# MaurizioFD/RecSys2019_DeepLearning_Evaluation

Hardware: AMD Instinct MI355X
Metric: BPR-MF SGD samples/sec (k=128, batch 1000) + ItemKNN cosine build sec on ML-20M-shaped URM (higher is better)
Workload: dtype f32; 1 GPU; BPR-MF epoch (139 mini-batches x 1000 on-device samples), k=128, sgd, on synthetic ml20m URM 138493x26744 nnz=20001422; replicas (one independent model per GPU); batch_size=1000, n_factors=128, parallelism=replicas x1

## Files before the change

recsys2019_deeplearning_evaluation_amd/csrc/mf_batch.cuh:

```cuda
#pragma once

namespace mi355rec {
namespace {

template <class T, int VEC> struct alignas(sizeof(T) * VEC) Chunk { T v[VEC]; };

template <class T, int VEC>
__device__ __forceinline__ Chunk<T, VEC> load_chunk(const T *row, int chunk, bool ok) {
    Chunk<T, VEC> r = *reinterpret_cast<const Chunk<T, VEC> *>(row + (size_t)(ok ? chunk : 0) * VEC);
#pragma unroll
    for (int e = 0; e < VEC; ++e) r.v[e] = ok ? r.v[e] : (T)0;
    return r;
}

template <class T, class P> __device__ __forceinline__ void adam_powers(const P &p, long long t, T &pw1, T &pw2) {
    pw1 = (T)1;
    pw2 = (T)1;
    if (p.sgd_mode == MI355REC_ADAM) {
        pw1 = (T)(1.0 - pow(p.beta_1_d, (double)t));
        pw2 = (T)(1.0 - pow(p.beta_2_d, (double)t));
    }
}

template <class T> struct MuRequest { MuState<T> st; T part; };

template <class T>
__device__ __forceinline__ MuRequest<T> global_bias_request(const MfParams<T> &p, const int prev, int lane) {
    MuRequest<T> r;
    r.st = p.mu_state[prev];
    r.part = p.mu_acc[prev * MU_SLOTS + lane];
    return r;
}

template <class T>
__device__ __forceinline__ T global_bias_finish(const MfParams<T> &p, MuRequest<T> r, long long gb, const int at, bool writer, int lane) {
    const int cur = at % 3, nxt = (at + 1) % 3;
    MuState<T> st = r.st;
    const T sum = wave_sum(r.part);
    if (gb > 0) {
        T pw1, pw2;
        adam_powers(p, gb, pw1, pw2);
        const T step = adapt_cell(p, sum * p.inv_batch, st.c1, st.c2, pw1, pw2);
        st.mu += p.lr * step;
    }
    if (writer) {
        if (lane == 0) p.mu_state[cur] = st;
        p.mu_acc[nxt * MU_SLOTS + lane] = (T)0;
    }
    return st.mu;
}

template <class T>
__device__ __forceinline__ T global_bias_at(const MfParams<T> &p, long long gb, const int at, bool writer, int lane) {
    return global_bias_finish(p, global_bias_request(p, (at + 2) % 3, lane), gb, at, writer, lane);
}

template <class T, int VEC, int KI, bool BPR> struct Rows {
    Chunk<T, VEC> A[KI], B[KI], C[BPR ? KI : 1];
    T bu, bi;
};

template <class T, int VEC, int LPR, int KI, bool BPR>
__device__ __forceinline__ Rows<T, VEC, KI, BPR> load_rows(const MfParams<T> &p, const int4 rec, int li, const bool (&cok)[KI],
                                                           bool bias) {
    Rows<T, VEC, KI, BPR> r;
    const int k = p.k;
    const T *Wu = ((rec.w >> 2) & 1 ? p.U1 : p.U0) + (size_t)rec.x * k;
    const T *Hi = ((rec.w >> 3) & 1 ? p.V1 : p.V0) + (size_t)rec.y * k;
    const T *Hj = ((rec.w >> 4) & 1 ? p.V1 : p.V0) + (size_t)(BPR ? rec.z : 0) * k;
#pragma unroll
    for (int c = 0; c < KI; ++c) {
        r.A[c] = load_chunk<T, VEC>(Wu, c * LPR + li, cok[c]);
        r.B[c] = load_chunk<T, VEC>(Hi, c * LPR + li, cok[c]);
        if (BPR) r.C[c] = load_chunk<T, VEC>(Hj, c * LPR + li, cok[c]);
    }
    r.bu = (T)0;
    r.bi = (T)0;
    if (bias) {
        r.bu = ((rec.w >> 2) & 1 ? p.bu1 : p.bu0)[rec.x];
        r.bi = ((rec.w >> 3) & 1 ? p.bi1 : p.bi0)[rec.y];
    }
    return r;
}

template <int ALGO, class T, int VEC, int LPR, int KI, bool ARGS_HERE>
__device__ __forceinline__ void mf_batch_body(const MfParams<T> &p, const int batch_local, const int wg, const int wv, const int tpb,
                                              const TaskHeader *hdr, const int4 *slot, const bool stamps) {
    constexpr int G = 64 / LPR;
    constexpr bool BPR = ALGO == MI355REC_MF_BPR;
    using Ch = Chunk<T, VEC>;
    using R = Rows<T, VEC, KI, BPR>;
    const int lane = threadIdx.x & 63;
    const unsigned long long tk0 = stamps ? stamp() : 0ull;
    const TaskHeader *hp = hdr + min(wv, tpb - 1);
    const int8v hd = *reinterpret_cast<const int8v *>(hp);
    int4 slot_rec = make_int4(0, 0, 0, 0);
    if constexpr (BPR && G > 1) slot_rec = slot[(size_t)min(wv, tpb - 1) * 3 + max(lane / LPR - 1, 0)];
    if constexpr (ARGS_HERE) {
        asm volatile("" ::"s"(p.ticks), "s"(p.use_bias), "s"(p.sgd_mode), "s"(p.state), "s"(p.mu_state), "s"(p.mu_acc), "s"(p.k), "s"(p.U0),
                     "s"(p.U1), "s"(p.V0), "s"(p.V1), "s"(p.recs));
    }
    const bool bias = !BPR && p.use_bias;
    long long gb = batch_local;
    long long batch_base = 0;
    MuRequest<T> mu_req;
    mu_req.st = MuState<T>{};
    mu_req.part = (T)0;
    if constexpr (!BPR) {
        int zero;
        asm volatile("v_mov_b32 %0, 0" : "=v"(zero));
        batch_base = (&p.state->batch_base)[zero];
        mu_req = global_bias_request(p, (batch_local + 2) % 3 + zero, lane);
    }
    if constexpr (!ARGS_HERE) asm volatile("" ::"s"(p.k), "s"(p.U0), "s"(p.U1), "s"(p.V0), "s"(p.V1), "s"(p.recs));
    if constexpr (BPR) {
        if (p.sgd_mode == MI355REC_ADAM) gb += p.state->batch_base;
    } else {
        gb += batch_base;
    }
    const int4 h0 = make_int4(hd[0], hd[1], hd[2], hd[3]), h1 = make_int4(hd[4], hd[5], hd[6], hd[7]);
    const bool active = (h0.y & LEN_MASK) != 0 && wv < tpb;
    __shared__ T s_mu[4];
    __shared__ T s_wide[4][LPR * KI * VEC];
    __shared__ T s_wide_bias[4];
    T mu_term = (T)0;
    T mu_eff = (T)0;
    unsigned long long tk1 = 0, tk2 = 0, tk3 = 0, tk4 = 0, tk5 = 0;
    if (p.ticks) tk1 = stamp();
    if (bias && !active) mu_eff = global_bias_finish(p, mu_req, gb, batch_local, wv == 0, lane);
    if (active) {
        const int entry = h0.x, len = h0.y & LEN_MASK, own_par = (unsigned)h0.y >> 31, start = h0.z;
        const bool wide = (h0.y & META_WIDE) != 0;
        const int part = (h0.y >> 28) & 3;
        const int base = wide ? part * G : 0, step = wide ? 4 * G : G;
        const int g = lane / LPR, li = lane % LPR;
        const int k = p.k, chunks = k / VEC;
        bool cok[KI];
#pragma unroll
        for (int c = 0; c < KI; ++c) cok[c] = c * LPR + li < chunks;
        const int iters = len > base ? (len - base + step - 1) / step : 0;
        int4 rec = h1;
        const bool pair = BPR && G > 1 && h0.w == 1;
        T sg_first = (T)0;
        if (BPR && G > 1 && h0.w == 1) {
            if (g != 0) rec = slot_rec;
        } else if (G > 1 && len > 1) {
            const int4 r = p.recs[start + min(base + g, len - 1)];
            if (g != 0) rec = r;
        }
        const int4 rec_first = rec;
        int4 rec_n = rec;
        if (iters > 1) rec_n = p.recs[start + min(base + step + g, len - 1)];
        R rows = load_rows<T, VEC, LPR, KI, BPR>(p, rec, li, cok, bias);
        if (bias) mu_eff = global_bias_finish(p, mu_req, gb, batch_local, wv == 0, lane);
        T pw1, pw2;
        adam_powers(p, gb + 1, pw1, pw2);

        Ch acc[KI], own[KI];
#pragma unroll
        for (int c = 0; c < KI; ++c)
#pragma unroll
            for (int e = 0; e < VEC; ++e) { acc[c].v[e] = (T)0; own[c].v[e] = (T)0; }
        T bias_acc = (T)0, own_bias = (T)0;
        double loss = 0.0;

        for (int it = 0; it < iters; ++it) {
            const int idx = base + it * step + g;
            const bool valid = idx < len;
            int4 rec_nn = rec_n;
            if (it + 2 < iters) rec_nn = p.recs[start + min(idx + 2 * step, len - 1)];
            R rows_n = rows;
            if (it + 1 < iters) rows_n = load_rows<T, VEC, LPR, KI, BPR>(p, rec_n, li, cok, bias);

            const int role = rec.w & 3;
            T dot = (T)0;
#pragma unroll
            for (int c = 0; c < KI; ++c)
#pragma unroll
                for (int e = 0; e < VEC; ++e)
                    dot = fused_add(rows.A[c].v[e], BPR ? diff_of(rows.B[c].v[e], rows.C[c].v[e]) : rows.B[c].v[e], dot);
            dot = group_sum<LPR>(dot);
            if (p.ticks && it == 0) {
                asm volatile("" ::"v"(dot));
                tk2 = stamp();
            }
            if (BPR) {
                const T x = dot;
                const T sg = sigmoid_of_minus(x);
                if (it == 0) sg_first = sg;
                if (valid && role == ROLE_U && li == 0) loss += (double)x * (double)x;
#pragma unroll
                for (int c = 0; c < KI; ++c)
#pragma unroll
                    for (int e = 0; e < VEC; ++e) {
                        const T a = rows.A[c].v[e], b = rows.B[c].v[e], cc = rows.C[c].v[e];
                        const T gU = grad_term(sg, diff_of(b, cc), p.user_reg, a);
                        const T gI = grad_term(sg, a, p.positive_reg, b);
                        const T gJ = grad_term(sg, -a, p.negative_reg, cc);
                        const T gr = role == ROLE_U ? gU : (role == ROLE_I ? gI : gJ);
                        acc[c].v[e] += valid ? gr : (T)0;
                        if (it == 0) own[c].v[e] = role == ROLE_U ? a : (role == ROLE_I ? b : cc);
                    }
            } else {
                T pred = dot;
                if (bias) pred += mu_eff + rows.bu + rows.bi;
                const T err = (T)__int_as_float(rec.z) - pred;
                if (valid && role == ROLE_U) {
                    if (li == 0) loss += (double)err * (double)err;
                    if (bias) mu_term += err - p.bias_reg * mu_eff;
                }
                if (bias && valid) bias_acc += err - p.bias_reg * (role == ROLE_U ? rows.bu : rows.bi);
                if (it == 0) own_bias = role == ROLE_U ? rows.bu : rows.bi;
#pragma unroll
                for (int c = 0; c < KI; ++c)
#pragma unroll
                    for (int e = 0; e < VEC; ++e) {
                        const T a = rows.A[c].v[e], b = rows.B[c].v[e];
                        const T gU = grad_term(err, b, p.user_reg, a);
                        const T gI = grad_term(err, a, p.positive_reg, b);
                        const T gr = role == ROLE_U ? gU : gI;
                        acc[c].v[e] += valid ? gr : (T)0;
                        if (it == 0) own[c].v[e] = role == ROLE_U ? a : b;
                    }
            }
            rec = rec_n;
            rec_n = rec_nn;
            rows = rows_n;
        }
        if (G > 1 && !pair) {
#pragma unroll
            for (int c = 0; c < KI; ++c)
#pragma unroll
                for (int e = 0; e < VEC; ++e) acc[c].v[e] = cross_group_sum<LPR>(acc[c].v[e]);
            if (bias) bias_acc = cross_group_sum<LPR>(bias_acc);
        }
        if (bias) {
            mu_term = li == 0 ? mu_term : (T)0;
            mu_term = wave_sum(mu_term);
        }
        if (li == 0 && loss != 0.0) atomicAdd(&p.loss_slots[wv * 4 + g], loss);
        if (p.ticks) tk3 = stamp();
        if (wide) {
            if (g == 0) {
#pragma unroll
                for (int c = 0; c < KI; ++c)
#pragma unroll
                    for (int e = 0; e < VEC; ++e) s_wide[part][(c * VEC + e) * LPR + li] = acc[c].v[e];
                if (li == 0) s_wide_bias[part] = bias_acc;
            }
            __syncthreads();
            if (part == 0 && g == 0) {
#pragma unroll
                for (int c = 0; c < KI; ++c)
#pragma unroll
                    for (int e = 0; e < VEC; ++e) {
                        const int at = (c * VEC + e) * LPR + li;
                        acc[c].v[e] = ((s_wide[0][at] + s_wide[1][at]) + s_wide[2][at]) + s_wide[3][at];
                    }
                bias_acc = ((s_wide_bias[0] + s_wide_bias[1]) + s_wide_bias[2]) + s_wide_bias[3];
            }
        }
        if ((g == 0 || pair) && (!wide || part == 0)) {
            const int own_entry = pair ? rec_first.x : entry;
            const int own_buf = pair ? (rec_first.w >> 2) & 1 : own_par;
            const bool is_item = own_entry >= p.n_users;
            const int row = is_item ? own_entry - p.n_users : own_entry;
            T *Wn = (is_item ? (own_buf ? p.V0 : p.V1) : (own_buf ? p.U0 : p.U1)) + (size_t)row * k;
            T *c1 = (is_item ? p.c1V : p.c1U) + (size_t)row * k, *c2 = (is_item ? p.c2V : p.c2U) + (size_t)row * k;
#pragma unroll
            for (int c = 0; c < KI; ++c) {
                if (!cok[c]) continue;
                const size_t at = (size_t)(c * LPR + li) * VEC;
                Ch m1, m2, out;
                if (p.sgd_mode != MI355REC_SGD) m1 = *reinterpret_cast<const Ch *>(c1 + at);
                if (p.sgd_mode == MI355REC_ADAM) m2 = *reinterpret_cast<const Ch *>(c2 + at);
#pragma unroll
                for (int e = 0; e < VEC; ++e) {
                    const T gm = mean_of(acc[c].v[e], p.inv_batch);
                    const T step = adapt_cell(p, gm, m1.v[e], m2.v[e], pw1, pw2);
                    out.v[e] = moved(own[c].v[e], p.lr, step);
                }
                *reinterpret_cast<Ch *>(Wn + at) = out;
                if (p.sgd_mode != MI355REC_SGD) *reinterpret_cast<Ch *>(c1 + at) = m1;
                if (p.sgd_mode == MI355REC_ADAM) *reinterpret_cast<Ch *>(c2 + at) = m2;
            }
            if (bias && li == 0) {
                T *bn = is_item ? (own_buf ? p.bi0 : p.bi1) : (own_buf ? p.bu0 : p.bu1);
                T *b1 = is_item ? p.c1_bi : p.c1_bu, *b2 = is_item ? p.c2_bi : p.c2_bu;
                const T step = adapt(p, bias_acc * p.inv_batch, b1, b2, (size_t)row, pw1, pw2);
                bn[row] = own_bias + p.lr * step;
            }
        }
        if (p.ticks) tk4 = stamp();
        const int also = BPR && (len == 1 || pair) ? (rec_first.w >> 5) & 3 : 0;
        if (BPR && also) {
#pragma unroll
            for (int e = 1; e <= 2; ++e) {
                if (!(also & e) || !(pair || g == e % G)) continue;
                const int item = e == 1 ? rec_first.y : rec_first.z;
                const int cur = (rec_first.w >> (e == 1 ? 3 : 4)) & 1;
                T *Wn = (cur ? p.V0 : p.V1) + (size_t)item * k;
                T *c1 = p.c1V + (size_t)item * k, *c2 = p.c2V + (size_t)item * k;
#pragma unroll
                for (int c = 0; c < KI; ++c) {
                    if (!cok[c]) continue;
                    const size_t at = (size_t)(c * LPR + li) * VEC;
                    Ch m1, m2, out;
                    if (p.sgd_mode != MI355REC_SGD) m1 = *reinterpret_cast<const Ch *>(c1 + at);
                    if (p.sgd_mode == MI355REC_ADAM) m2 = *reinterpret_cast<const Ch *>(c2 + at);
#pragma unroll
                    for (int v = 0; v < VEC; ++v) {
                        const T a = rows.A[c].v[v], b = rows.B[c].v[v], cc = rows.C[c].v[v];
                        const T gr = e == 1 ? grad_term(sg_first, a, p.positive_reg, b) : grad_term(sg_first, -a, p.negative_reg, cc);
                        const T gm = mean_of((T)0 + gr, p.inv_batch);
                        const T step = adapt_cell(p, gm, m1.v[v], m2.v[v], pw1, pw2);
                        out.v[v] = moved(e == 1 ? b : cc, p.lr, step);
                    }
                    *reinterpret_cast<Ch *>(Wn + at) = out;
                    if (p.sgd_mode != MI355REC_SGD) *reinterpret_cast<Ch *>(c1 + at) = m1;
                    if (p.sgd_mode == MI355REC_ADAM) *reinterpret_cast<Ch *>(c2 + at) = m2;
                }
            }
        }
    }
    if (p.ticks) tk5 = stamp();
    if (bias) {
        if (lane == 0) s_mu[threadIdx.x >> 6] = mu_term;
        __syncthreads();
        if (threadIdx.x == 0) {
            const T sum = (s_mu[0] + s_mu[1]) + (s_mu[2] + s_mu[3]);
            if (sum != (T)0) atomicAdd(&p.mu_acc[(batch_local % 3) * MU_SLOTS + (wg & (MU_SLOTS - 1))], sum);
        }
    }
    if (p.ticks && lane == 0 && wv < tpb) {
        unsigned long long *o = p.ticks + (size_t)wv * 8;
        o[0] = tk0; o[1] = tk1; o[2] = tk2; o[3] = tk3; o[4] = stamp(); o[5] = (unsigned long long)(h0.y & LEN_MASK);
        o[6] = tk4; o[7] = tk5;
    }
}

template <int ALGO, class T, int VEC, int LPR, int KI, bool PLAIN_SGD>
__global__ __launch_bounds__(256) void mf_batch_kernel(const TaskHeader *hdr, const int4 *slot, const int tasks_per_batch, const int wg_base,
                                                       const int wg_stride, const int stamps, const MfParams<T> p, const int batch_local) {
    if constexpr (PLAIN_SGD) __builtin_assume(p.sgd_mode == MI355REC_SGD);
    const int wv = __builtin_amdgcn_readfirstlane((blockIdx.x * wg_stride + wg_base) * 4 + (threadIdx.x >> 6));
    mf_batch_body<ALGO, T, VEC, LPR, KI, true>(p, batch_local, blockIdx.x, wv, tasks_per_batch, hdr, slot, stamps != 0);
}

template <class P> __device__ __forceinline__ P *as_global(P *q) {
    const unsigned long long bits = (unsigned long long)q;
    return (P *)(__attribute__((address_space(1))) P *)bits;
}
template <class T> __device__ __forceinline__ void globalize(MfParams<T> &p) {
    p.indptr = as_global(p.indptr); p.indices = as_global(p.indices); p.data = as_global(p.data);
    p.U0 = as_global(p.U0); p.U1 = as_global(p.U1); p.V0 = as_global(p.V0); p.V1 = as_global(p.V1);
    p.bu0 = as_global(p.bu0); p.bu1 = as_global(p.bu1); p.bi0 = as_global(p.bi0); p.bi1 = as_global(p.bi1);
    p.c1U = as_global(p.c1U); p.c2U = as_global(p.c2U); p.c1V = as_global(p.c1V); p.c2V = as_global(p.c2V);
    p.c1_bu = as_global(p.c1_bu); p.c2_bu = as_global(p.c2_bu); p.c1_bi = as_global(p.c1_bi); p.c2_bi = as_global(p.c2_bi);
    p.mu_state = as_global(p.mu_state); p.mu_acc = as_global(p.mu_acc);
    p.loss_slots = as_global(p.loss_slots); p.state = as_global(p.state);
    p.su = as_global(p.su); p.si = as_global(p.si); p.sj = as_global(p.sj); p.sr = as_global(p.sr);
    p.tasks = as_global(p.tasks); p.recs = as_global(p.recs); p.ticks = as_global(p.ticks); p.used = as_global(p.used);
    p.slot_recs = as_global(p.slot_recs);
}

template <int ALGO, class T, int VEC, int LPR, int KI, bool PLAIN_SGD>
__global__ __launch_bounds__(256, (PLAIN_SGD && ALGO == MI355REC_MF_BPR && sizeof(T) == 4 && LPR == 32) ? 6 : 1) void mf_group_batch_kernel(const MfParams<T> *__restrict__ table, const int batch_local) {
    MfParams<T> p = table[blockIdx.y];
    globalize(p);
    if constexpr (PLAIN_SGD) __builtin_assume(p.sgd_mode == MI355REC_SGD);
    const int used = p.used ? p.used[batch_local] : p.tasks_per_batch;
    const TaskHeader *hdr = p.tasks + (size_t)batch_local * p.tasks_per_batch;
    const int4 *slot = p.slot_recs + (size_t)batch_local * p.slot_rec_stride;
    for (int wg = blockIdx.x; wg * 4 < used; wg += gridDim.x) {
        const int wv = __builtin_amdgcn_readfirstlane((wg * p.wg_stride + p.wg_base) * 4 + (threadIdx.x >> 6));
        mf_batch_body<ALGO, T, VEC, LPR, KI, false>(p, batch_local, wg, wv, p.tasks_per_batch, hdr, slot, p.ticks != nullptr);
    }
}
__device__ __forceinline__ void globalize(FastSchedParams &f) {
    f.su = as_global(f.su); f.si = as_global(f.si); f.sj = as_global(f.sj); f.sr = as_global(f.sr);
    f.touched = as_global(f.touched); f.par = as_global(f.par); f.sorted_slot = as_global(f.sorted_slot); f.qtask = as_global(f.qtask);
    f.used = as_global(f.used); f.tasks = as_global(f.tasks); f.recs = as_global(f.recs); f.slot_recs = as_global(f.slot_recs);
}
template <int ALGO, class T>
__global__ __launch_bounds__(256) void mf_group_sample_kernel(const MfParams<T> *__restrict__ table) {
    MfParams<T> p = table[blockIdx.y];
    globalize(p);
    mf_sample_body<ALGO, T>(p);
}
template <class T>
__global__ void mf_group_epoch_advance_kernel(const MfParams<T> *table, const int n_models) {
    const int m = blockIdx.x * blockDim.x + threadIdx.x;
    if (m < n_models) table[m].state->epoch += 1;
}
__global__ __launch_bounds__(SCHED_THREADS) void mf_group_sched_sort_kernel(const FastSchedParams *__restrict__ table) {
    FastSchedParams f = table[blockIdx.y];
    globalize(f);
    mf_sched_sort_body(f, blockIdx.x);
}
__global__ __launch_bounds__(256) void mf_group_sched_emit_kernel(const FastSchedParams *__restrict__ table) {
    FastSchedParams f = table[blockIdx.z];
    globalize(f);
    mf_sched_emit_body(f);
}
__global__ __launch_bounds__(256) void mf_group_sched_finish_kernel(const FastSchedParams *__restrict__ table) {
    FastSchedParams f = table[blockIdx.y];
    globalize(f);
    mf_sched_finish_body(f);
}

template <int ALGO, class T>
__global__ __launch_bounds__(256) void mf_batch_generic_kernel(const MfParams<T> p, const int batch_local) {
    constexpr bool BPR = ALGO == MI355REC_MF_BPR;
    constexpr int KMAX_REG = 8;
    const int lane = threadIdx.x & 63;
    const int wv = __builtin_amdgcn_readfirstlane((blockIdx.x * p.wg_stride + p.wg_base) * 4 + (threadIdx.x >> 6));
    const TaskHeader *hp = p.tasks + ((size_t)batch_local * p.tasks_per_batch + min(wv, p.tasks_per_batch - 1));
    const int4 h0 = *reinterpret_cast<const int4 *>(hp);
    const bool active = (h0.y & LEN_MASK) != 0 && wv < p.tasks_per_batch;
    const bool bias = !BPR && p.use_bias;
    __shared__ T s_mu[4];
    T mu_term = (T)0;
    if (active || bias) {
        const long long gb = p.state->batch_base + batch_local;
        T mu_eff = (T)0;
        if (bias) mu_eff = global_bias_at(p, gb, batch_local, wv == 0, lane);
        if (active) {
            const int entry = h0.x, len = h0.y & LEN_MASK, own_par = (unsigned)h0.y >> 31, start = h0.z;
            const int k = p.k;
            T pw1, pw2;
            adam_powers(p, gb + 1, pw1, pw2);
            T acc[KMAX_REG];
#pragma unroll
            for (int c = 0; c < KMAX_REG; ++c) acc[c] = (T)0;
            T bias_acc = (T)0;
            double loss = 0.0;
            for (int idx = 0; idx < len; ++idx) {
                const int4 rec = idx == 0 ? hp->rec0 : p.recs[start + idx];
                const int role = rec.w & 3;
                const T *Wu = ((rec.w >> 2) & 1 ? p.U1 : p.U0) + (size_t)rec.x * k;
                const T *Hi = ((rec.w >> 3) & 1 ? p.V1 : p.V0) + (size_t)rec.y * k;
                const T *Hj = ((rec.w >> 4) & 1 ? p.V1 : p.V0) + (size_t)(BPR ? rec.z : 0) * k;
                T dot = (T)0;
                for (int f = lane; f < k; f += 64) dot += BPR ? Wu[f] * (Hi[f] - Hj[f]) : Wu[f] * Hi[f];
                dot = wave_sum(dot);
                if (BPR) {
                    const T sg = sigmoid_of_minus(dot);
                    if (role == ROLE_U) loss += (double)dot * (double)dot;
#pragma unroll
                    for (int c = 0; c < KMAX_REG; ++c) {
                        const int f = lane + 64 * c;
                        if (f < k) {
                            const T a = Wu[f], b = Hi[f], cc = Hj[f];
                            acc[c] += role == ROLE_U ? sg * (b - cc) - p.user_reg * a
                                                     : (role == ROLE_I ? sg * a - p.positive_reg * b : sg * (-a) - p.negative_reg * cc);
                        }
                    }
                } else {
                    T bu_v = (T)0, bi_v = (T)0;
                    if (bias) {
                        bu_v = ((rec.w >> 2) & 1 ? p.bu1 : p.bu0)[rec.x];
                        bi_v = ((rec.w >> 3) & 1 ? p.bi1 : p.bi0)[rec.y];
                    }
                    const T err = __int_as_float(rec.z) - (dot + (bias ? mu_eff + bu_v + bi_v : (T)0));
                    if (role == ROLE_U) {
                        loss += (double)err * (double)err;
                        if (bias) mu_term += err - p.bias_reg * mu_eff;
                    }
                    if (bias) bias_acc += err - p.bias_reg * (role == ROLE_U ? bu_v : bi_v);
#pragma unroll
                    for (int c = 0; c < KMAX_REG; ++c) {
                        const int f = lane + 64 * c;
                        if (f < k) {
                            const T a = Wu[f], b = Hi[f];
                            acc[c] += role == ROLE_U ? err * b - p.user_reg * a : err * a - p.positive_reg * b;
                        }
                    }
                }
            }
            if (lane == 0 && loss != 0.0) p.loss_slots[wv * 4] += loss;
            const bool is_item = entry >= p.n_users;
            const int row = is_item ? entry - p.n_users : entry;
            const T *Wo = (is_item ? (own_par ? p.V1 : p.V0) : (own_par ? p.U1 : p.U0)) + (size_t)row * k;
            T *Wn = (is_item ? (own_par ? p.V0 : p.V1) : (own_par ? p.U0 : p.U1)) + (size_t)row * k;
            T *c1 = is_item ? p.c1V : p.c1U, *c2 = is_item ? p.c2V : p.c2U;
#pragma unroll
            for (int c = 0; c < KMAX_REG; ++c) {
                const int f = lane + 64 * c;
                if (f < k) {
                    const T step = adapt(p, acc[c] * p.inv_batch, c1, c2, (size_t)row * k + f, pw1, pw2);
                    Wn[f] = Wo[f] + p.lr * step;
                }
            }
            if (bias && lane == 0) {
                const T *bo = is_item ? (own_par ? p.bi1 : p.bi0) : (own_par ? p.bu1 : p.bu0);
                T *bn = is_item ? (own_par ? p.bi0 : p.bi1) : (own_par ? p.bu0 : p.bu1);
                T *b1 = is_item ? p.c1_bi : p.c1_bu, *b2 = is_item ? p.c2_bi : p.c2_bu;
                const T step = adapt(p, bias_acc * p.inv_batch, b1, b2, (size_t)row, pw1, pw2);
                bn[row] = bo[row] + p.lr * step;
            }
            mu_term = lane == 0 ? mu_term : (T)0;
        }
    }
    if (bias) {
        if (lane == 0) s_mu[threadIdx.x >> 6] = mu_term;
        __syncthreads();
        if (threadIdx.x == 0) {
            const T sum = (s_mu[0] + s_mu[1]) + (s_mu[2] + s_mu[3]);
            if (sum != (T)0) atomicAdd(&p.mu_acc[(batch_local % 3) * MU_SLOTS + (blockIdx.x & (MU_SLOTS - 1))], sum);
        }
    }
}

template <class T, bool PACK>
__global__ __launch_bounds__(256) void mf_shard_rows_kernel(const MfParams<T> p, const int batch_local, const int rank, const int world,
                                                            const int slots_per_rank, T *slab) {
    const int lane = threadIdx.x & 63;
    const int slot = blockIdx.x * 4 + (threadIdx.x >> 6);
    if (slot >= p.tasks_per_batch) return;
    const int wg = slot >> 2, owner = wg % world;
    if ((owner == rank) != PACK) return;
    const TaskHeader *hd = p.tasks + ((size_t)batch_local * p.tasks_per_batch + slot);
    const int meta = hd->meta;
    if ((meta & LEN_MASK) == 0) return;
    if ((meta & META_WIDE) && ((meta >> 28) & 3) != 0) return;
    const int entry = hd->entry, own_par = (unsigned)meta >> 31;
    const bool is_item = entry >= p.n_users;
    const int row = is_item ? entry - p.n_users : entry;
    T *Wn = (is_item ? (own_par ? p.V0 : p.V1) : (own_par ? p.U0 : p.U1)) + (size_t)row * p.k;
    const int local = (wg / world) * 4 + (slot & 3);
    T *at = slab + ((size_t)(PACK ? 0 : owner) * slots_per_rank + local) * p.k;
    for (int e = lane; e < p.k; e += 64) {
        if (PACK) at[e] = Wn[e];
        else Wn[e] = at[e];
    }
}

template <class T, class O>
__global__ __launch_bounds__(256) void mf_gather_rows_kernel(const T *b0, const T *b1, const unsigned char *par, long long n_rows,
                                                             int k, O *out) {
    const long long t = blockIdx.x * (long long)blockDim.x + threadIdx.x;
    if (t >= n_rows * k) return;
    const long long row = t / k;
    out[t] = (O)(par[row] ? b1[t] : b0[t]);
}
template <class T, class O>
__global__ void mf_final_mu_kernel(const MfParams<T> p, O *out) {
    const int lane = threadIdx.x & 63;
    const T mu = global_bias_at(p, p.state->batch_base, 0, false, lane);
    if (threadIdx.x == 0) out[0] = (O)mu;
}

}
}
```

Before: 226.8 million samples/s.

## Specialize single-sample BPR tasks and hoist optimizer-state loads and write addresses

Splits the per-task body into a lambda that is compiled twice. One copy is a single-iteration path for the common pair or length-one task, the other keeps the general loop. Optimizer moment loads (m1/m2), bias-state loads and all write-back addresses are hoisted ahead of the dot-product loop so their latency overlaps compute. Side item updates reuse gradients captured on the first iteration instead of being recomputed. This raises register pressure, and the longer live ranges plus the explicit waitcnt could reduce occupancy.

```diff
diff --git a/recsys2019_deeplearning_evaluation_amd/csrc/mf_batch.cuh b/recsys2019_deeplearning_evaluation_amd/csrc/mf_batch.cuh
--- a/recsys2019_deeplearning_evaluation_amd/csrc/mf_batch.cuh
+++ b/recsys2019_deeplearning_evaluation_amd/csrc/mf_batch.cuh
@@ -81,6 +81,15 @@
         r.bi = ((rec.w >> 3) & 1 ? p.bi1 : p.bi0)[rec.y];
     }
     return r;
+}
+
+template <class P> __device__ __forceinline__ P *as_global(P *q) {
+    const unsigned long long bits = (unsigned long long)q;
+    return (P *)(__attribute__((address_space(1))) P *)bits;
+}
+template <class P> __device__ __forceinline__ P *held(P *q) {
+    asm volatile("" : "+v"(q));
+    return as_global(q);
 }
 
 template <int ALGO, class T, int VEC, int LPR, int KI, bool ARGS_HERE>
@@ -98,7 +107,8 @@
     if constexpr (BPR && G > 1) slot_rec = slot[(size_t)min(wv, tpb - 1) * 3 + max(lane / LPR - 1, 0)];
     if constexpr (ARGS_HERE) {
         asm volatile("" ::"s"(p.ticks), "s"(p.use_bias), "s"(p.sgd_mode), "s"(p.state), "s"(p.mu_state), "s"(p.mu_acc), "s"(p.k), "s"(p.U0),
-                     "s"(p.U1), "s"(p.V0), "s"(p.V1), "s"(p.recs));
+                     "s"(p.U1), "s"(p.V0), "s"(p.V1), "s"(p.recs),
+                     "s"(p.n_users), "s"(p.lr), "s"(p.user_reg), "s"(p.positive_reg), "s"(p.negative_reg), "s"(p.inv_batch), "s"(p.loss_slots));
     }
     const bool bias = !BPR && p.use_bias;
     long long gb = batch_local;
@@ -130,37 +140,124 @@
     if (bias && !active) mu_eff = global_bias_finish(p, mu_req, gb, batch_local, wv == 0, lane);
     if (active) {
         const int entry = h0.x, len = h0.y & LEN_MASK, own_par = (unsigned)h0.y >> 31, start = h0.z;
-        const bool wide = (h0.y & META_WIDE) != 0;
-        const int part = (h0.y >> 28) & 3;
-        const int base = wide ? part * G : 0, step = wide ? 4 * G : G;
         const int g = lane / LPR, li = lane % LPR;
         const int k = p.k, chunks = k / VEC;
         bool cok[KI];
 #pragma unroll
         for (int c = 0; c < KI; ++c) cok[c] = c * LPR + li < chunks;
-        const int iters = len > base ? (len - base + step - 1) / step : 0;
-        int4 rec = h1;
         const bool pair = BPR && G > 1 && h0.w == 1;
-        T sg_first = (T)0;
-        if (BPR && G > 1 && h0.w == 1) {
-            if (g != 0) rec = slot_rec;
-        } else if (G > 1 && len > 1) {
+        const int h1x = h1.x, h1y = h1.y, h1z = h1.z, h1w = h1.w, srx = slot_rec.x, sry = slot_rec.y, srz = slot_rec.z, srw = slot_rec.w;
+        auto task = [&](auto one_sample) __attribute__((always_inline)) {
+        constexpr bool ONE = decltype(one_sample)::value;
+        const bool wide = !ONE && (h0.y & META_WIDE) != 0;
+        const int part = (h0.y >> 28) & 3;
+        const int base = wide ? part * G : 0;
+        int4 rec = make_int4(h1x, h1y, h1z, h1w);
+        if constexpr (ONE) {
+            const bool other = pair && g != 0;
+            rec = make_int4(other ? srx : h1x, other ? sry : h1y, other ? srz : h1z, other ? srw : h1w);
+        } else if (G > 1) {
             const int4 r = p.recs[start + min(base + g, len - 1)];
             if (g != 0) rec = r;
         }
+        asm volatile("" : "+v"(rec.x), "+v"(rec.y), "+v"(rec.z), "+v"(rec.w));
         const int4 rec_first = rec;
+        R rows = load_rows<T, VEC, LPR, KI, BPR>(p, rec, li, cok, bias);
+        constexpr int LG = G == 1 ? 0 : (G == 2 ? 1 : (G == 4 ? 2 : (G == 8 ? 3 : 4)));
+        static_assert((1 << LG) == G, "lane groups per wavefront: a power of two");
+        const int step = wide ? 4 * G : G;
+        const int iters = ONE ? 1 : (len > base ? (len - base + step - 1) >> (wide ? LG + 2 : LG) : 0);
         int4 rec_n = rec;
         if (iters > 1) rec_n = p.recs[start + min(base + step + g, len - 1)];
-        R rows = load_rows<T, VEC, LPR, KI, BPR>(p, rec, li, cok, bias);
+        const bool writer = (g == 0 || pair) && (!wide || part == 0);
+        const int own_entry = pair ? rec_first.x : entry;
+        const int own_buf = pair ? (rec_first.w >> 2) & 1 : own_par;
+        const bool is_item = own_entry >= p.n_users;
+        const int row = is_item ? own_entry - p.n_users : own_entry;
+        const size_t lane_at = (size_t)li * VEC;
+        T *Wn = (is_item ? (own_buf ? p.V0 : p.V1) : (own_buf ? p.U0 : p.U1)) + (size_t)row * k + lane_at;
+        const int also = BPR && ONE ? (rec_first.w >> 5) & 3 : 0;
+        bool take[2] = {false, false};
+        T *Wt[2] = {nullptr, nullptr};
+        if constexpr (BPR) {
+#pragma unroll
+            for (int e = 1; e <= 2; ++e) {
+                take[e - 1] = (also & e) && (pair || g == e % G);
+                const int item = e == 1 ? rec_first.y : rec_first.z;
+                const int cur = (rec_first.w >> (e == 1 ? 3 : 4)) & 1;
+                Wt[e - 1] = (cur ? p.V0 : p.V1) + (size_t)item * k + lane_at;
+            }
+        }
+        unsigned loss_at = (unsigned)(wv * 4 + g) * (unsigned)sizeof(double);
+        Ch m1o[KI], m2o[KI], m1t[2][KI], m2t[2][KI];
+        T mb1 = (T)0, mb2 = (T)0;
+#pragma unroll
+        for (int c = 0; c < KI; ++c)
+#pragma unroll
+            for (int e = 0; e < VEC; ++e) {
+                m1o[c].v[e] = m2o[c].v[e] = (T)0;
+                m1t[0][c].v[e] = m2t[0][c].v[e] = m1t[1][c].v[e] = m2t[1][c].v[e] = (T)0;
+            }
+        T *c1o = nullptr, *c2o = nullptr, *c1t[2] = {nullptr, nullptr}, *c2t[2] = {nullptr, nullptr};
+        T *bn = nullptr, *b1 = nullptr, *b2 = nullptr;
+        if (bias) {
+            bn = (is_item ? (own_buf ? p.bi0 : p.bi1) : (own_buf ? p.bu0 : p.bu1)) + row;
+            b1 = (is_item ? p.c1_bi : p.c1_bu) + row;
+            b2 = (is_item ? p.c2_bi : p.c2_bu) + row;
+        }
+        if (p.sgd_mode != MI355REC_SGD) {
+            const bool adam = p.sgd_mode == MI355REC_ADAM;
+            c1o = (is_item ? p.c1V : p.c1U) + (size_t)row * k;
+            c2o = (is_item ? p.c2V : p.c2U) + (size_t)row * k;
+#pragma unroll
+            for (int c = 0; c < KI; ++c) m1o[c] = load_chunk<T, VEC>(c1o, c * LPR + li, cok[c]);
+            if constexpr (BPR) {
+#pragma unroll
+                for (int e = 0; e < 2; ++e) {
+                    const size_t at = (size_t)(e == 0 ? rec_first.y : rec_first.z) * k;
+                    c1t[e] = p.c1V + at;
+                    c2t[e] = p.c2V + at;
+#pragma unroll
+                    for (int c = 0; c < KI; ++c) m1t[e][c] = load_chunk<T, VEC>(c1t[e], c * LPR + li, cok[c]);
+                }
+            }
+            int zero = 0;
+            if (bias) {
+                asm volatile("v_mov_b32 %0, 0" : "=v"(zero));
+                mb1 = b1[zero];
+            }
+            if (adam) {
+#pragma unroll
+                for (int c = 0; c < KI; ++c) m2o[c] = load_chunk<T, VEC>(c2o, c * LPR + li, cok[c]);
+                if constexpr (BPR) {
+#pragma unroll
+                    for (int e = 0; e < 2; ++e)
+#pragma unroll
+                        for (int c = 0; c < KI; ++c) m2t[e][c] = load_chunk<T, VEC>(c2t[e], c * LPR + li, cok[c]);
+                }
+                if (bias) mb2 = b2[zero];
+            }
+            c1o += lane_at;
+            c2o += lane_at;
+            c1t[0] += lane_at; c1t[1] += lane_at;
+            c2t[0] += lane_at; c2t[1] += lane_at;
+        }
         if (bias) mu_eff = global_bias_finish(p, mu_req, gb, batch_local, wv == 0, lane);
         T pw1, pw2;
         adam_powers(p, gb + 1, pw1, pw2);
+        Wn = held(Wn);
+        if constexpr (BPR) { Wt[0] = held(Wt[0]); Wt[1] = held(Wt[1]); }
+        asm volatile("" : "+v"(loss_at));
 
         Ch acc[KI], own[KI];
+        Ch firstB[KI], firstC[KI], firstI[KI], firstJ[KI];
 #pragma unroll
         for (int c = 0; c < KI; ++c)
 #pragma unroll
-            for (int e = 0; e < VEC; ++e) { acc[c].v[e] = (T)0; own[c].v[e] = (T)0; }
+            for (int e = 0; e < VEC; ++e) {
+                acc[c].v[e] = (T)0; own[c].v[e] = (T)0;
+                firstB[c].v[e] = firstC[c].v[e] = firstI[c].v[e] = firstJ[c].v[e] = (T)0;
+            }
         T bias_acc = (T)0, own_bias = (T)0;
         double loss = 0.0;
 
@@ -187,7 +284,6 @@
             if (BPR) {
                 const T x = dot;
                 const T sg = sigmoid_of_minus(x);
-                if (it == 0) sg_first = sg;
                 if (valid && role == ROLE_U && li == 0) loss += (double)x * (double)x;
 #pragma unroll
                 for (int c = 0; c < KI; ++c)
@@ -199,7 +295,10 @@
                         const T gJ = grad_term(sg, -a, p.negative_reg, cc);
                         const T gr = role == ROLE_U ? gU : (role == ROLE_I ? gI : gJ);
                         acc[c].v[e] += valid ? gr : (T)0;
-                        if (it == 0) own[c].v[e] = role == ROLE_U ? a : (role == ROLE_I ? b : cc);
+                        if (it == 0) {
+                            own[c].v[e] = role == ROLE_U ? a : (role == ROLE_I ? b : cc);
+                            firstB[c].v[e] = b; firstC[c].v[e] = cc; firstI[c].v[e] = gI; firstJ[c].v[e] = gJ;
+                        }
                     }
             } else {
                 T pred = dot;
@@ -238,7 +337,8 @@
             mu_term = li == 0 ? mu_term : (T)0;
             mu_term = wave_sum(mu_term);
         }
-        if (li == 0 && loss != 0.0) atomicAdd(&p.loss_slots[wv * 4 + g], loss);
+        __builtin_amdgcn_s_waitcnt(0x0f70);
+        if (li == 0 && loss != 0.0) atomicAdd(reinterpret_cast<double *>(reinterpret_cast<char *>(p.loss_slots) + loss_at), loss);
         if (p.ticks) tk3 = stamp();
         if (wide) {
             if (g == 0) {
@@ -260,68 +360,66 @@
                 bias_acc = ((s_wide_bias[0] + s_wide_bias[1]) + s_wide_bias[2]) + s_wide_bias[3];
             }
         }
-        if ((g == 0 || pair) && (!wide || part == 0)) {
-            const int own_entry = pair ? rec_first.x : entry;
-            const int own_buf = pair ? (rec_first.w >> 2) & 1 : own_par;
-            const bool is_item = own_entry >= p.n_users;
-            const int row = is_item ? own_entry - p.n_users : own_entry;
-            T *Wn = (is_item ? (own_buf ? p.V0 : p.V1) : (own_buf ? p.U0 : p.U1)) + (size_t)row * k;
-            T *c1 = (is_item ? p.c1V : p.c1U) + (size_t)row * k, *c2 = (is_item ? p.c2V : p.c2U) + (size_t)row * k;
+        Ch out[KI], outt[2][KI];
+#pragma unroll
+        for (int c = 0; c < KI; ++c)
+#pragma unroll
+            for (int e = 0; e < VEC; ++e) {
+                const T gm = mean_of(acc[c].v[e], p.inv_batch);
+                const T st = adapt_cell(p, gm, m1o[c].v[e], m2o[c].v[e], pw1, pw2);
+                out[c].v[e] = moved(own[c].v[e], p.lr, st);
+            }
+        if (BPR && (p.sgd_mode == MI355REC_SGD || also)) {
+#pragma unroll
+            for (int t = 0; t < 2; ++t)
+#pragma unroll
+                for (int c = 0; c < KI; ++c)
+#pragma unroll
+                    for (int v = 0; v < VEC; ++v) {
+                        const T gr = t == 0 ? firstI[c].v[v] : firstJ[c].v[v];
+                        const T gm = mean_of((T)0 + gr, p.inv_batch);
+                        const T st = adapt_cell(p, gm, m1t[t][c].v[v], m2t[t][c].v[v], pw1, pw2);
+                        outt[t][c].v[v] = moved(t == 0 ? firstB[c].v[v] : firstC[c].v[v], p.lr, st);
+                    }
+        }
+        if constexpr (BPR && ONE) {
+#pragma unroll
+            for (int c = 0; c < KI; ++c)
+#pragma unroll
+                for (int e = 0; e < VEC; ++e) asm volatile("" ::"v"(outt[0][c].v[e]), "v"(outt[1][c].v[e]));
+        }
+        if (writer) {
 #pragma unroll
             for (int c = 0; c < KI; ++c) {
                 if (!cok[c]) continue;
-                const size_t at = (size_t)(c * LPR + li) * VEC;
-                Ch m1, m2, out;
-                if (p.sgd_mode != MI355REC_SGD) m1 = *reinterpret_cast<const Ch *>(c1 + at);
-                if (p.sgd_mode == MI355REC_ADAM) m2 = *reinterpret_cast<const Ch *>(c2 + at);
-#pragma unroll
-                for (int e = 0; e < VEC; ++e) {
-                    const T gm = mean_of(acc[c].v[e], p.inv_batch);
-                    const T step = adapt_cell(p, gm, m1.v[e], m2.v[e], pw1, pw2);
-                    out.v[e] = moved(own[c].v[e], p.lr, step);
-                }
-                *reinterpret_cast<Ch *>(Wn + at) = out;
-                if (p.sgd_mode != MI355REC_SGD) *reinterpret_cast<Ch *>(c1 + at) = m1;
-                if (p.sgd_mode == MI355REC_ADAM) *reinterpret_cast<Ch *>(c2 + at) = m2;
+                *reinterpret_cast<Ch *>(Wn + c * LPR * VEC) = out[c];
+                if (p.sgd_mode != MI355REC_SGD) *reinterpret_cast<Ch *>(c1o + c * LPR * VEC) = m1o[c];
+                if (p.sgd_mode == MI355REC_ADAM) *reinterpret_cast<Ch *>(c2o + c * LPR * VEC) = m2o[c];
             }
             if (bias && li == 0) {
-                T *bn = is_item ? (own_buf ? p.bi0 : p.bi1) : (own_buf ? p.bu0 : p.bu1);
-                T *b1 = is_item ? p.c1_bi : p.c1_bu, *b2 = is_item ? p.c2_bi : p.c2_bu;
-                const T step = adapt(p, bias_acc * p.inv_batch, b1, b2, (size_t)row, pw1, pw2);
-                bn[row] = own_bias + p.lr * step;
+                const T st = adapt_cell(p, bias_acc * p.inv_batch, mb1, mb2, pw1, pw2);
+                *bn = own_bias + p.lr * st;
+                if (p.sgd_mode != MI355REC_SGD) *b1 = mb1;
+                if (p.sgd_mode == MI355REC_ADAM) *b2 = mb2;
             }
         }
         if (p.ticks) tk4 = stamp();
-        const int also = BPR && (len == 1 || pair) ? (rec_first.w >> 5) & 3 : 0;
-        if (BPR && also) {
-#pragma unroll
-            for (int e = 1; e <= 2; ++e) {
-                if (!(also & e) || !(pair || g == e % G)) continue;
-                const int item = e == 1 ? rec_first.y : rec_first.z;
-                const int cur = (rec_first.w >> (e == 1 ? 3 : 4)) & 1;
-                T *Wn = (cur ? p.V0 : p.V1) + (size_t)item * k;
-                T *c1 = p.c1V + (size_t)item * k, *c2 = p.c2V + (size_t)item * k;
+        if constexpr (BPR) {
+#pragma unroll
+            for (int t = 0; t < 2; ++t) {
+                if (!take[t]) continue;
 #pragma unroll
                 for (int c = 0; c < KI; ++c) {
                     if (!cok[c]) continue;
-                    const size_t at = (size_t)(c * LPR + li) * VEC;
-                    Ch m1, m2, out;
-                    if (p.sgd_mode != MI355REC_SGD) m1 = *reinterpret_cast<const Ch *>(c1 + at);
-                    if (p.sgd_mode == MI355REC_ADAM) m2 = *reinterpret_cast<const Ch *>(c2 + at);
-#pragma unroll
-                    for (int v = 0; v < VEC; ++v) {
-                        const T a = rows.A[c].v[v], b = rows.B[c].v[v], cc = rows.C[c].v[v];
-                        const T gr = e == 1 ? grad_term(sg_first, a, p.positive_reg, b) : grad_term(sg_first, -a, p.negative_reg, cc);
-                        const T gm = mean_of((T)0 + gr, p.inv_batch);
-                        const T step = adapt_cell(p, gm, m1.v[v], m2.v[v], pw1, pw2);
-                        out.v[v] = moved(e == 1 ? b : cc, p.lr, step);
-                    }
-                    *reinterpret_cast<Ch *>(Wn + at) = out;
-                    if (p.sgd_mode != MI355REC_SGD) *reinterpret_cast<Ch *>(c1 + at) = m1;
-                    if (p.sgd_mode == MI355REC_ADAM) *reinterpret_cast<Ch *>(c2 + at) = m2;
+                    *reinterpret_cast<Ch *>(Wt[t] + c * LPR * VEC) = outt[t][c];
+                    if (p.sgd_mode != MI355REC_SGD) *reinterpret_cast<Ch *>(c1t[t] + c * LPR * VEC) = m1t[t][c];
+                    if (p.sgd_mode == MI355REC_ADAM) *reinterpret_cast<Ch *>(c2t[t] + c * LPR * VEC) = m2t[t][c];
                 }
             }
         }
+        };
+        if (__builtin_expect(pair || len == 1, true)) task(std::true_type{});
+        else task(std::false_type{});
     }
     if (p.ticks) tk5 = stamp();
     if (bias) {
@@ -347,10 +445,6 @@
     mf_batch_body<ALGO, T, VEC, LPR, KI, true>(p, batch_local, blockIdx.x, wv, tasks_per_batch, hdr, slot, stamps != 0);
 }
 
-template <class P> __device__ __forceinline__ P *as_global(P *q) {
-    const unsigned long long bits = (unsigned long long)q;
-    return (P *)(__attribute__((address_space(1))) P *)bits;
-}
 template <class T> __device__ __forceinline__ void globalize(MfParams<T> &p) {
     p.indptr = as_global(p.indptr); p.indices = as_global(p.indices); p.data = as_global(p.data);
     p.U0 = as_global(p.U0); p.U1 = as_global(p.U1); p.V0 = as_global(p.V0); p.V1 = as_global(p.V1);
```

New measurement: 228.9 million samples/s, median of 6. No clear change (+0.9%).
